# abowman6/CBET_RayTracing_3D

Measured on AMD Instinct MI355X. Metric: ray-steps/sec, OMEGA 60-beam 256^3 sweep, higher is better.
Workload: dtype f64

## Files before the change

cbet_raytracing_3d_amd/build.py:

```python
import os
import shutil
import subprocess
import sys

PKG = os.path.dirname(os.path.abspath(__file__))
ROOT = os.path.dirname(PKG)
CSRC = os.path.join(PKG, "csrc")
LIB_DIR = os.path.join(PKG, "lib")
LIB_PATH = os.path.join(LIB_DIR, "libcbet_mi355x.so")
SOURCES = ["cbet_kernels.hip", "cbet_trace_window.hip", "cbet_trace_exit.hip", "cbet_grid_kernels.hip", "cbet_sph_modes.hip",
           "cbet_target.hip", "cbet_flow.hip", "cbet_abi.cpp", "cbet_host.cpp", "cbet_output.cpp", "cbet_sph_host.cpp", "cbet_target_host.cpp"]
HEADERS = [os.path.join(CSRC, "cbet_device.h"), os.path.join(CSRC, "cbet_relocate.h"), os.path.join(CSRC, "cbet_trace_common.h"), os.path.join(CSRC, "cbet_target_model.h"), os.path.join(ROOT, "include", "cbet_mi355x.h"),
           os.path.join(ROOT, "include", "cbet_omega_beams.h")]

FLAGS = ["-O3", "-std=c++17", "--offload-arch=gfx950", "-ffp-contract=off", "-fPIC", "-shared",
         "-Wall", "-Wextra", "-Wno-unused-result", "-mllvm", "-structurizecfg-skip-uniform-regions=true"]


def hipcc():
    exe = shutil.which("hipcc") or "/opt/rocm/bin/hipcc"
    if not os.path.exists(exe):
        raise RuntimeError("hipcc not found (need ROCm to build the gfx950 library)")
    return exe


def is_stale():
    if not os.path.exists(LIB_PATH):
        return True
    built = os.path.getmtime(LIB_PATH)
    deps = [os.path.join(CSRC, s) for s in SOURCES] + HEADERS + [os.path.abspath(__file__),
                                                                os.path.join(ROOT, "tools", "cbet_gpu.cpp"),
                                                                os.path.join(ROOT, "tools", "cbet_reference_shaped.cpp"),
                                                                os.path.join(ROOT, "include", "cbet_reference_api.hpp")]
    return any(os.path.getmtime(d) > built for d in deps)


def build(force=False, verbose=False, extra_flags=()):
    if not force and not is_stale():
        return LIB_PATH
    os.makedirs(LIB_DIR, exist_ok=True)
    cmd = [hipcc()] + FLAGS + list(extra_flags) + [
        "-I", os.path.join(ROOT, "include"), "-I", CSRC,
        "-o", LIB_PATH] + [os.path.join(CSRC, s) for s in SOURCES] + ["-lrccl"]
    if verbose:
        print(" ".join(cmd), flush=True)
    run = subprocess.run(cmd, stderr=subprocess.PIPE, text=True)
    sys.stderr.write(run.stderr)
    if run.returncode != 0 and "structurizecfg-skip-uniform-regions" in run.stderr:
        print("build: this hipcc does not know -structurizecfg-skip-uniform-regions; building without it", flush=True)
        k = cmd.index("-structurizecfg-skip-uniform-regions=true")
        subprocess.check_call(cmd[:k - 1] + cmd[k + 1:])
    elif run.returncode != 0:
        raise subprocess.CalledProcessError(run.returncode, cmd)
    build_cli(verbose)
    build_ref_shaped(verbose)
    return LIB_PATH


CLI_PATH = os.path.join(PKG, "lib", "cbet-gpu")


def build_cli(verbose=False):
    cmd = ["g++", "-O2", "-std=c++17", "-I", os.path.join(ROOT, "include"),
           os.path.join(ROOT, "tools", "cbet_gpu.cpp"), "-o", CLI_PATH,
           "-L", LIB_DIR, "-lcbet_mi355x", "-Wl,-rpath,$ORIGIN", "-Wl,-rpath-link," + "/opt/rocm/lib"]
    if verbose:
        print(" ".join(cmd), flush=True)
    subprocess.check_call(cmd)
    return CLI_PATH


REF_SHAPED_PATH = os.path.join(PKG, "lib", "cbet-ref-shaped")


def build_ref_shaped(verbose=False):
    cmd = [hipcc(), "-O2", "-std=c++17", "-I", os.path.join(ROOT, "include"),
           os.path.join(ROOT, "tools", "cbet_reference_shaped.cpp"), "-o", REF_SHAPED_PATH,
           "-L", LIB_DIR, "-lcbet_mi355x", "-Wl,-rpath,$ORIGIN"]
    if verbose:
        print(" ".join(cmd), flush=True)
    subprocess.check_call(cmd)
    return REF_SHAPED_PATH


def build_variant(name, extra_flags=(), verbose=False):
    out_dir = os.path.join(ROOT, "build_alt")
    os.makedirs(out_dir, exist_ok=True)
    out = os.path.join(out_dir, "libcbet_%s.so" % name)
    cmd = [hipcc()] + FLAGS + list(extra_flags) + ["-I", os.path.join(ROOT, "include"), "-I", CSRC, "-o", out] + \
        [os.path.join(CSRC, s) for s in SOURCES] + ["-lrccl"]
    if verbose:
        print(" ".join(cmd), flush=True)
    subprocess.check_call(cmd)
    return out


if __name__ == "__main__":
    if len(sys.argv) > 2 and sys.argv[1] == "--variant":
        print(build_variant(sys.argv[2], sys.argv[3:], verbose=True))
    else:
        print(build(force="--force" in sys.argv, verbose=True))
```

cbet_raytracing_3d_amd/csrc/cbet_kernels.hip:

```cpp
#include <hip/hip_runtime.h>

#include "cbet_trace_common.h"

namespace cbet {
namespace {

__device__ __forceinline__ void interp_table2(const double *y1, const double *y2, const double *x, const double xp,
                                              int n, double &o1, double &o2)
{
    const bool ascending = x[0] <= x[n - 1];
    if (ascending ? (xp <= x[0]) : (xp >= x[0])) { o1 = y1[0]; o2 = y2[0]; return; }
    if (ascending ? (xp >= x[n - 1]) : (xp <= x[n - 1])) { o1 = y1[n - 1]; o2 = y2[n - 1]; return; }
    unsigned lo = 0, hi = n - 1, mid = (lo + hi) >> 1;
    while (lo < hi - 1) {
        const bool go_low = ascending ? (x[mid] >= xp) : !(x[mid] <= xp);
        if (go_low) hi = mid; else lo = mid;
        mid = (lo + hi) >> 1;
    }
    const double dx = x[mid + 1] - x[mid], t = xp - x[mid];
    o1 = y1[mid] + (y1[mid + 1] - y1[mid]) / dx * t;
    o2 = y2[mid] + (y2[mid + 1] - y2[mid]) / dx * t;
}

__device__ __forceinline__ void node_plasma(const TabulateArgs &a, const double *s_r, const double *s_ne, const double *s_te,
                                            int i, int j, int k, double &ed, double &kap)
{
    const double xc = i * a.dx + a.xmin, yc = j * a.dy + a.ymin, zc = k * a.dz + a.zmin;
    const double rho = sqrt(xc * xc + yc * yc + zc * zc);
    double etemp;
    interp_table2(s_ne, s_te, s_r, rho, a.nprofile, ed, etemp);
    const double eta = 5.2e-5 * 10.0 / (etemp * sqrt(etemp));
    const double nuei = (1e6 * ed * (kEc * kEc) / kMe) * eta;
    kap = ed / a.ncrit * nuei * a.dt;
}

__global__ void __launch_bounds__(256) k_tabulate(const TabulateArgs a)
{
    extern __shared__ double s_prof[];
    double *s_r = s_prof, *s_ne = s_prof + a.nprofile, *s_te = s_prof + 2 * a.nprofile;
    for (int i = threadIdx.x; i < a.nprofile; i += blockDim.x) {
        s_r[i] = a.r[i];
        s_ne[i] = a.ne[i];
        s_te[i] = a.te[i];
    }
    __syncthreads();
    const long total = (long)a.nx * a.ny * a.nz;
    const long stride = (long)gridDim.x * blockDim.x;
    for (long idx = (long)blockIdx.x * blockDim.x + threadIdx.x; idx < total; idx += stride) {
        const int k = (int)(idx % a.nz);
        const long ij = idx / a.nz;
        const int j = (int)(ij % a.ny);
        const int i = (int)(ij / a.ny);
        double ed, kap;
        node_plasma(a, s_r, s_ne, s_te, i, j, k, ed, kap);
        a.ne3d[idx] = ed;
        a.kap3d[idx] = kap;
    }
}

__global__ void __launch_bounds__(256) k_step_table(const StepTableArgs a)
{
    const long total = (long)a.nx * a.ny * a.nz;
    const long stride = (long)gridDim.x * blockDim.x;
    const long sY = a.nz, sX = (long)a.ny * a.nz;
    for (long idx = (long)blockIdx.x * blockDim.x + threadIdx.x; idx < total; idx += stride) {
        const int k = (int)(idx % a.nz);
        const long ij = idx / a.nz;
        const int j = (int)(ij % a.ny);
        const int i = (int)(ij / a.ny);
        const long oxm = (i == 0) ? 0 : ((i == a.nx - 1) ? -2 * sX : -sX), oxp = (i == 0) ? 2 * sX : ((i == a.nx - 1) ? 0 : sX);
        const long oym = (j == 0) ? 0 : ((j == a.ny - 1) ? -2 * sY : -sY), oyp = (j == 0) ? 2 * sY : ((j == a.ny - 1) ? 0 : sY);
        const long ozm = (k == 0) ? 0 : ((k == a.nz - 1) ? -2 : -1), ozp = (k == 0) ? 2 : ((k == a.nz - 1) ? 0 : 1);
        StepRecord r;
        r.kx = a.xconst * (a.ne3d[idx + oxp] - a.ne3d[idx + oxm]);
        r.ky = a.yconst * (a.ne3d[idx + oyp] - a.ne3d[idx + oym]);
        r.kz = a.zconst * (a.ne3d[idx + ozp] - a.ne3d[idx + ozm]);
        r.kap = a.kap3d[idx];
        a.rec[idx] = r;
    }
}

constexpr int kPrTY = 8, kPrTZ = 64, kPrXC = 16, kPrThreads = 256;
constexpr int kPrPZ = kPrTZ + 2;
constexpr int kPrPlane = (kPrTY + 2) * kPrPZ;
constexpr int kPrTile = kPrTY * kPrTZ;
constexpr int kPrItems = kPrTile + 2 * kPrTZ + 2 * kPrTY;

__global__ void __launch_bounds__(kPrThreads) k_plasma_records(const PlasmaRecordsArgs a)
{
    extern __shared__ double s_prof[];
    const TabulateArgs &t = a.t;
    double *s_r = s_prof, *s_ne = s_prof + t.nprofile, *s_te = s_prof + 2 * t.nprofile;
    double *s_ring = s_prof + 3 * t.nprofile;
    double *s_kap = s_ring + 3 * kPrPlane;
    const int tid = threadIdx.x;
    for (int i = tid; i < t.nprofile; i += kPrThreads) {
        s_r[i] = t.r[i];
        s_ne[i] = t.ne[i];
        s_te[i] = t.te[i];
    }
    __syncthreads();
    const int nx = t.nx, ny = t.ny, nz = t.nz;
    const int k0 = max(0, min((int)blockIdx.x * kPrTZ, nz - kPrTZ));
    const int j0 = max(0, min((int)blockIdx.y * kPrTY, ny - kPrTY));
    const int x0 = (int)blockIdx.z * kPrXC, x1 = min(x0 + kPrXC, nx);
    const int pa = x0 == 0 ? 0 : min(x0 - 1, nx - 3);
    const int pb = x1 == nx ? nx : max(x1 + 1, 3);

    auto emit = [&](int i, int xl, int xh) {
        const double *lo = s_ring + (xl % 3) * kPrPlane, *hi = s_ring + (xh % 3) * kPrPlane, *mid = s_ring + (i % 3) * kPrPlane;
        const double *kap = s_kap + (i % 3) * kPrTile;
        for (int q = tid; q < 2 * kPrTile; q += kPrThreads) {
            const int n = q >> 1, jr = n / kPrTZ, kr = n % kPrTZ;
            const int j = j0 + jr, k = k0 + kr;
            if (j >= ny || k >= nz) continue;
            const int c = (jr + 1) * kPrPZ + kr + 1;
            double v0, v1;
            if ((q & 1) == 0) {
                const int ym = (j == 0) ? 0 : ((j == ny - 1) ? -2 : -1), yp = (j == 0) ? 2 : ((j == ny - 1) ? 0 : 1);
                v0 = a.xconst * (hi[c] - lo[c]);
                v1 = a.yconst * (mid[c + yp * kPrPZ] - mid[c + ym * kPrPZ]);
            } else {
                const int zm = (k == 0) ? 0 : ((k == nz - 1) ? -2 : -1), zp = (k == 0) ? 2 : ((k == nz - 1) ? 0 : 1);
                v0 = a.zconst * (mid[c + zp] - mid[c + zm]);
                v1 = kap[n];
            }
            const long idx = ((long)i * ny + j) * nz + k;
            reinterpret_cast<double2 *>(a.rec + idx)[q & 1] = make_double2(v0, v1);
        }
    };

    for (int p = pa; p < pb; ++p) {
        const bool own_plane = p >= x0 && p < x1;
        double *ring = s_ring + (p % 3) * kPrPlane;
        for (int n = tid; n < (own_plane ? kPrItems : kPrTile); n += kPrThreads) {
            int jj, kk;
            if (n < kPrTile) {
                jj = 1 + n / kPrTZ; kk = 1 + n % kPrTZ;
            } else if (n < kPrTile + 2 * kPrTZ) {
                const int h = n - kPrTile;
                jj = h < kPrTZ ? 0 : kPrTY + 1; kk = 1 + h % kPrTZ;
            } else {
                const int h = n - kPrTile - 2 * kPrTZ;
                kk = h < kPrTY ? 0 : kPrTZ + 1; jj = 1 + h % kPrTY;
            }
            const int j = j0 + jj - 1, k = k0 + kk - 1;
            if (j < 0 || j >= ny || k < 0 || k >= nz) continue;
            double ed, kap;
            if (own_plane && n < kPrTile) {
                node_plasma(t, s_r, s_ne, s_te, p, j, k, ed, kap);
                s_kap[(p % 3) * kPrTile + n] = kap;
                const long idx = ((long)p * ny + j) * nz + k;
                t.ne3d[idx] = ed;
                t.kap3d[idx] = kap;
            } else {
                node_plasma(t, s_r, s_ne, s_te, p, j, k, ed, kap);
            }
            ring[jj * kPrPZ + kk] = ed;
        }
        __syncthreads();
        if (p == 2 && x0 == 0) emit(0, 0, 2);
        if (p - 1 >= 1 && p - 1 >= x0 && p - 1 < x1) emit(p - 1, p - 2, p);
        if (p == nx - 1 && x1 == nx) emit(nx - 1, nx - 3, nx - 1);
        __syncthreads();
    }
}

template <int WL>
struct LdsWindow {
    static constexpr int W = 1 << WL;
    static constexpr int NSLOT = W * W * W;
    double *val;
    unsigned *tag;
    const TraceArgs *args;

    __device__ __forceinline__ unsigned slot(int i, int j, int k) const
    {
        return (unsigned)((((i & (W - 1)) << WL) | (j & (W - 1))) << WL | (k & (W - 1)));
    }
    __device__ __forceinline__ void clear(int lane)
    {
        for (int s = lane; s < NSLOT; s += kWave) {
            val[s] = 0.0;
            tag[s] = kEmptyTag;
        }
    }
    __device__ __forceinline__ void add(unsigned s, double w)
    {
        if (CBET_AUDIT(*args, s < (unsigned)NSLOT))
            __hip_atomic_fetch_add(&val[s], w, __ATOMIC_RELAXED, __HIP_MEMORY_SCOPE_WORKGROUP);
    }
    __device__ __forceinline__ int flush(int lane, double *edep)
    {
        int n = 0;
        for (int s = lane; s < NSLOT; s += kWave) {
            const unsigned t = tag[s];
            if (t != kEmptyTag) {
                global_add(*args, &edep[t], val[s]);
                ++n;
            }
        }
        return n;
    }
};

template <int WL>
__device__ __forceinline__ void lds_deposit8(LdsWindow<WL> &win, bool pending, const unsigned (&slot)[8],
                                             const unsigned (&node)[8], const double (&w)[8],
                                             double *edep, int &n_evict)
{
    unsigned miss = 0;
    if (pending) {
        unsigned t[8];
#pragma unroll
        for (int c = 0; c < 8; ++c)
            t[c] = __hip_atomic_load(&win.tag[slot[c]], __ATOMIC_RELAXED, __HIP_MEMORY_SCOPE_WORKGROUP);
#pragma unroll
        for (int c = 0; c < 8; ++c) {
            if (t[c] == node[c])
                win.add(slot[c], w[c]);
            else
                miss |= 1u << c;
        }
    }
    if (!__any(miss != 0)) return;
    __builtin_amdgcn_wave_barrier();
#pragma unroll
    for (int c = 0; c < 8; ++c) {
        bool pend = (miss >> c) & 1u;
        while (__any(pend)) {
            unsigned t = 0;
            if (pend)
                t = __hip_atomic_load(&win.tag[slot[c]], __ATOMIC_RELAXED, __HIP_MEMORY_SCOPE_WORKGROUP);
            if (pend && t == node[c]) {
                win.add(slot[c], w[c]);
                pend = false;
            }
            __builtin_amdgcn_wave_barrier();
            if (pend) {
                unsigned expect = t;
                const bool won = __hip_atomic_compare_exchange_strong(
                    &win.tag[slot[c]], &expect, node[c], __ATOMIC_RELAXED, __ATOMIC_RELAXED,
                    __HIP_MEMORY_SCOPE_WORKGROUP);
                if (won) {
                    const unsigned long long old = __hip_atomic_exchange(
                        reinterpret_cast<unsigned long long *>(&win.val[slot[c]]),
                        (unsigned long long)__double_as_longlong(w[c]), __ATOMIC_RELAXED,
                        __HIP_MEMORY_SCOPE_WORKGROUP);
                    if (t != kEmptyTag) {
                        global_add(*win.args, &edep[t], __longlong_as_double((long long)old));
                        ++n_evict;
                    }
                    pend = false;
                }
            }
            __builtin_amdgcn_wave_barrier();
        }
    }
}

template <int DEPOSIT>
__global__ void __launch_bounds__(kWave) k_trace_simple(const TraceArgs a)
{
    constexpr int WL = 3;
    constexpr int NSLOT = DEPOSIT == 2 ? (1 << (3 * WL)) : 1;
    __shared__ double s_val[NSLOT];
    __shared__ unsigned s_tag[NSLOT];
    const int lane = threadIdx.x;
    int beam, patch;
    if (!work_item(a, blockIdx.x, beam, patch)) return;
    double *const edep = a.edep + (long)(beam - a.grid_beam0) * a.grid_stride;
    const bool absorb = a.absorption == 1;

    Ray s;
    const int li = patch * kWave + lane;
    const int pre_raynum = li < a.nlive ? a.live[li] : -1;
    bool alive = pre_raynum >= 0;
    if (alive) alive = launch_ray(a, beam, pre_raynum, s);
    const int launched = alive ? 1 : 0;

    const int nx = a.nx, ny = a.ny, nz = a.nz;
    const long sY = nz, sX = (long)ny * nz;
    const int sYh = a.sYh, sXh = a.sXh;
    int nsteps = 0, n_atomics = 0, n_evict = 0;
    unsigned wave_steps = 0;

    LdsWindow<WL> tagged{s_val, s_tag, &a};
    if (DEPOSIT == 2) {
        tagged.clear(lane);
        __syncthreads();
    }

    for (int tt = 0; tt < a.nt; ++tt) {
        if (__ballot(alive) == 0) break;
        ++wave_steps;
        unsigned slot[8] = {0, 0, 0, 0, 0, 0, 0, 0}, node[8] = {0, 0, 0, 0, 0, 0, 0, 0};
        double wgt[8] = {0, 0, 0, 0, 0, 0, 0, 0};
        if (alive) {
            const int im = (s.ci == 0) ? 0 : ((s.ci == nx - 1) ? nx - 3 : s.ci - 1);
            const int ip = (s.ci == 0) ? 2 : ((s.ci == nx - 1) ? nx - 1 : s.ci + 1);
            const int jm = (s.cj == 0) ? 0 : ((s.cj == ny - 1) ? ny - 3 : s.cj - 1);
            const int jp = (s.cj == 0) ? 2 : ((s.cj == ny - 1) ? ny - 1 : s.cj + 1);
            const int km = (s.ck == 0) ? 0 : ((s.ck == nz - 1) ? nz - 3 : s.ck - 1);
            const int kp = (s.ck == 0) ? 2 : ((s.ck == nz - 1) ? nz - 1 : s.ck + 1);
            auto ne_at = [&](int i, int j, int k) { return node_load<true>(a, a.ne3d, (unsigned)(i * sX + j * sY + k)); };
            s.vx -= a.xconst * (ne_at(ip, s.cj, s.ck) - ne_at(im, s.cj, s.ck));
            s.vy -= a.yconst * (ne_at(s.ci, jp, s.ck) - ne_at(s.ci, jm, s.ck));
            s.vz -= a.zconst * (ne_at(s.ci, s.cj, kp) - ne_at(s.ci, s.cj, km));
            s.px += s.vx * a.dt;
            s.py += s.vy * a.dt;
            s.pz += s.vz * a.dt;
            const double fx = (s.px - a.xmin) * a.inv_dx;
            const double fy = (s.py - a.ymin) * a.inv_dy;
            const double fz = (s.pz - a.zmin) * a.inv_dz;
            s.ci = relocate_loop(s.ci, fx, nx);
            s.cj = relocate_loop(s.cj, fy, ny);
            s.ck = relocate_loop(s.ck, fz, nz);
            double inc;
            if (absorb) {
                inc = node_load<true>(a, a.kap3d, (unsigned)(s.ci * sX + s.cj * sY + s.ck)) * s.uray;
                s.uray -= inc;
            } else {
                inc = s.uray;
            }
            const double ox = fx - s.ci - 0.5, oy = fy - s.cj - 0.5, oz = fz - s.ck - 0.5;
            const double dm = 1.0 - fabs(ox), dn = 1.0 - fabs(oy), dl = 1.0 - fabs(oz);
            const int X0 = s.ci + 1, X1 = X0 + (ox < 0 ? -1 : 1);
            const int Y0 = s.cj + 1, Y1 = Y0 + (oy < 0 ? -1 : 1);
            const int Z0 = s.ck + 1, Z1 = Z0 + (oz < 0 ? -1 : 1);
            const double Fx0 = 1.0 - dm, Fy0 = 1.0 - dn, Fz0 = 1.0 - dl;
            const double zy00 = Fz0 * Fy0, zy10 = dl * Fy0, zy01 = Fz0 * dn, zy11 = dl * dn;
            wgt[0] = zy00 * Fx0 * inc; wgt[1] = zy00 * dm * inc; wgt[2] = zy10 * Fx0 * inc; wgt[3] = zy10 * dm * inc;
            wgt[4] = zy01 * Fx0 * inc; wgt[5] = zy01 * dm * inc; wgt[6] = zy11 * Fx0 * inc; wgt[7] = zy11 * dm * inc;
            const int nX0 = X0 * sXh, nX1 = X1 * sXh, nY0 = Y0 * sYh, nY1 = Y1 * sYh;
            node[0] = nX0 + nY0 + Z0; node[1] = nX1 + nY0 + Z0; node[2] = nX0 + nY0 + Z1; node[3] = nX1 + nY0 + Z1;
            node[4] = nX0 + nY1 + Z0; node[5] = nX1 + nY1 + Z0; node[6] = nX0 + nY1 + Z1; node[7] = nX1 + nY1 + Z1;
            if (DEPOSIT == 1) {
#pragma unroll
                for (int c = 0; c < 8; ++c) global_add(a, &edep[node[c]], wgt[c]);
                n_atomics += 8;
            } else {
                slot[0] = tagged.slot(X0, Y0, Z0); slot[1] = tagged.slot(X1, Y0, Z0);
                slot[2] = tagged.slot(X0, Y0, Z1); slot[3] = tagged.slot(X1, Y0, Z1);
                slot[4] = tagged.slot(X0, Y1, Z0); slot[5] = tagged.slot(X1, Y1, Z0);
                slot[6] = tagged.slot(X0, Y1, Z1); slot[7] = tagged.slot(X1, Y1, Z1);
            }
            ++nsteps;
        }
        if (DEPOSIT == 2) lds_deposit8<WL>(tagged, alive, slot, node, wgt, edep, n_evict);
        if (alive) {
            const double *b = a.bounds;
            if (s.uray <= s.ustop || s.px < b[0] || s.px > b[1] || s.py < b[2] || s.py > b[3] || s.pz < b[4] || s.pz > b[5])
                alive = false;
        }
    }
    if (DEPOSIT == 2) {
        __syncthreads();
        n_atomics += tagged.flush(lane, edep) + n_evict;
    }
    const int tot_steps = wave_sum(nsteps), tot_rays = wave_sum(launched), tot_at = wave_sum(n_atomics),
              tot_ev = wave_sum(n_evict);
    if (lane == 0) {
        atomicAdd(&a.counters[kCntSteps], (unsigned long long)tot_steps);
        atomicAdd(&a.counters[kCntRays], (unsigned long long)tot_rays);
        atomicAdd(&a.counters[kCntGlobalAtomics], (unsigned long long)tot_at);
        atomicAdd(&a.counters[kCntEvictions], (unsigned long long)tot_ev);
        atomicAdd(&a.counters[kCntWaveSteps], (unsigned long long)wave_steps);
    }
}

#ifdef CBET_DEBUG_BOUNDS
__device__ unsigned long long g_audit_violations;
#endif

}

hipError_t launch_tabulate(const TabulateArgs &a, hipStream_t stream)
{
    const long total = (long)a.nx * a.ny * a.nz;
    long blocks = (total + 255) / 256;
    if (blocks > 256 * 16) blocks = 256 * 16;
    const size_t lds = sizeof(double) * 3 * (size_t)a.nprofile;
    hipLaunchKernelGGL(k_tabulate, dim3((unsigned)blocks), dim3(256), lds, stream, a);
    return hipGetLastError();
}

hipError_t launch_step_table(const StepTableArgs &a, hipStream_t stream)
{
    const long total = (long)a.nx * a.ny * a.nz;
    long blocks = (total + 255) / 256;
    if (blocks > 256 * 16) blocks = 256 * 16;
    hipLaunchKernelGGL(k_step_table, dim3((unsigned)blocks), dim3(256), 0, stream, a);
    return hipGetLastError();
}

size_t plasma_records_lds(int nprofile)
{
    return sizeof(double) * (3 * (size_t)nprofile + 3 * (size_t)kPrPlane + 3 * (size_t)kPrTile);
}

hipError_t launch_plasma_records(const PlasmaRecordsArgs &a, hipStream_t stream)
{
    const dim3 grid((unsigned)((a.t.nz + kPrTZ - 1) / kPrTZ), (unsigned)((a.t.ny + kPrTY - 1) / kPrTY),
                    (unsigned)((a.t.nx + kPrXC - 1) / kPrXC));
    hipLaunchKernelGGL(k_plasma_records, grid, dim3(kPrThreads), plasma_records_lds(a.t.nprofile), stream, a);
    return hipGetLastError();
}

hipError_t audit_violations(unsigned long long *out, bool reset, hipStream_t stream)
{
#ifdef CBET_DEBUG_BOUNDS
    hipError_t e = hipStreamSynchronize(stream);
    if (e != hipSuccess) return e;
    e = hipMemcpyFromSymbol(out, HIP_SYMBOL(g_audit_violations), sizeof *out);
    if (e == hipSuccess && reset) {
        const unsigned long long zero = 0;
        e = hipMemcpyToSymbol(HIP_SYMBOL(g_audit_violations), &zero, sizeof zero);
    }
    return e;
#else
    (void)out; (void)reset; (void)stream;
    return hipErrorNotSupported;
#endif
}

hipError_t launch_trace(const TraceArgs &a0, int variant, bool force_idx64, hipStream_t stream)
{
    TraceArgs a = a0;
#ifdef CBET_DEBUG_BOUNDS
    {
        const long cells = (long)(a.nx + 2) * a.sXh;
        a.audit_lo = a.edep;
        a.audit_hi = a.edep + (a.grid_stride ? a.grid_stride * (long)(a.beam_lo - a.grid_beam0 + a.nbeams_local) : cells);
        if (a.quantity != 0) a.audit_hi = a.edep + 4 * a.comp_stride;
        a.audit_nodes = (unsigned long long)a.nx * a.ny * a.nz;
        a.audit_hsize = (unsigned long long)a.hsize;
        hipError_t e = hipGetSymbolAddress((void **)&a.audit_count, HIP_SYMBOL(g_audit_violations));
        if (e != hipSuccess) return e;
    }
#endif
    if (variant == CBET_KERNEL_LDS_WINDOW) return launch_trace_window(a, force_idx64, stream);
    if (variant == kTraceExits) return launch_trace_exit(a, force_idx64, stream);
    const long waves = a.item_count;
    if (waves <= 0) return hipSuccess;
    const dim3 grid((unsigned)waves);
    if (variant == CBET_KERNEL_GLOBAL_ATOMICS) hipLaunchKernelGGL((k_trace_simple<1>), grid, dim3(kWave), 0, stream, a);
    else hipLaunchKernelGGL((k_trace_simple<2>), grid, dim3(kWave), 0, stream, a);
    return hipGetLastError();
}

}
```

Before: 167.3 billion.

## Replace binary-search profile interpolation with binned lookup and precomputed slopes

In the plasma-records kernel, the per-node binary search over the radial profile is replaced by a 1024-bin start-index table plus a short linear walk, with segment slopes precomputed in LDS. Halo nodes now compute only density, and the x/y squared terms are hoisted per plane. A fallback to the old search is kept for non-monotonic or degenerate profiles. It uses more LDS and adds setup work per block. Precomputed slopes change rounding slightly compared with the divide-per-lookup form.

```diff
diff --git a/cbet_raytracing_3d_amd/build.py b/cbet_raytracing_3d_amd/build.py
--- a/cbet_raytracing_3d_amd/build.py
+++ b/cbet_raytracing_3d_amd/build.py
@@ -10,7 +10,7 @@
 LIB_PATH = os.path.join(LIB_DIR, "libcbet_mi355x.so")
 SOURCES = ["cbet_kernels.hip", "cbet_trace_window.hip", "cbet_trace_exit.hip", "cbet_grid_kernels.hip", "cbet_sph_modes.hip",
            "cbet_target.hip", "cbet_flow.hip", "cbet_abi.cpp", "cbet_host.cpp", "cbet_output.cpp", "cbet_sph_host.cpp", "cbet_target_host.cpp"]
-HEADERS = [os.path.join(CSRC, "cbet_device.h"), os.path.join(CSRC, "cbet_relocate.h"), os.path.join(CSRC, "cbet_trace_common.h"), os.path.join(CSRC, "cbet_target_model.h"), os.path.join(ROOT, "include", "cbet_mi355x.h"),
+HEADERS = [os.path.join(CSRC, "cbet_device.h"), os.path.join(CSRC, "cbet_relocate.h"), os.path.join(CSRC, "cbet_profile_search.h"), os.path.join(CSRC, "cbet_trace_common.h"), os.path.join(CSRC, "cbet_target_model.h"), os.path.join(ROOT, "include", "cbet_mi355x.h"),
            os.path.join(ROOT, "include", "cbet_omega_beams.h")]
 
 FLAGS = ["-O3", "-std=c++17", "--offload-arch=gfx950", "-ffp-contract=off", "-fPIC", "-shared",
diff --git a/cbet_raytracing_3d_amd/csrc/cbet_kernels.hip b/cbet_raytracing_3d_amd/csrc/cbet_kernels.hip
--- a/cbet_raytracing_3d_amd/csrc/cbet_kernels.hip
+++ b/cbet_raytracing_3d_amd/csrc/cbet_kernels.hip
@@ -1,5 +1,6 @@
 #include <hip/hip_runtime.h>
 
+#include "cbet_profile_search.h"
 #include "cbet_trace_common.h"
 
 namespace cbet {
@@ -85,21 +86,63 @@
 constexpr int kPrPlane = (kPrTY + 2) * kPrPZ;
 constexpr int kPrTile = kPrTY * kPrTZ;
 constexpr int kPrItems = kPrTile + 2 * kPrTZ + 2 * kPrTY;
+constexpr int kPrDoubles = 3 * kPrPlane + 3 * kPrTile;
+
+__device__ __forceinline__ void records_node_plasma(const TabulateArgs &a, const ProfileTables &prof, bool direct, double xy,
+                                                    int k, double &ed, double &kap)
+{
+    const double zc = k * a.dz + a.zmin;
+    const double rho = sqrt(xy + zc * zc);
+    double etemp;
+    if (direct) profile_interp2(prof, rho, ed, etemp);
+    else interp_table2(prof.y1, prof.y2, prof.x, rho, a.nprofile, ed, etemp);
+    const double eta = 5.2e-5 * 10.0 / (etemp * sqrt(etemp));
+    const double nuei = (1e6 * ed * (kEc * kEc) / kMe) * eta;
+    kap = ed / a.ncrit * nuei * a.dt;
+}
+
+__device__ __forceinline__ double records_node_ne(const TabulateArgs &a, const ProfileTables &prof, bool direct, double xy, int k)
+{
+    const double zc = k * a.dz + a.zmin;
+    const double rho = sqrt(xy + zc * zc);
+    if (direct) return profile_interp1(prof, rho);
+    double ed, etemp;
+    interp_table2(prof.y1, prof.y2, prof.x, rho, a.nprofile, ed, etemp);
+    return ed;
+}
 
 __global__ void __launch_bounds__(kPrThreads) k_plasma_records(const PlasmaRecordsArgs a)
 {
     extern __shared__ double s_prof[];
     const TabulateArgs &t = a.t;
-    double *s_r = s_prof, *s_ne = s_prof + t.nprofile, *s_te = s_prof + 2 * t.nprofile;
-    double *s_ring = s_prof + 3 * t.nprofile;
+    const int np = t.nprofile;
+    double *s_r = s_prof, *s_ne = s_prof + np, *s_te = s_prof + 2 * np;
+    double *s_sne = s_prof + 3 * np, *s_ste = s_prof + 4 * np;
+    double *s_ring = s_prof + 5 * np;
     double *s_kap = s_ring + 3 * kPrPlane;
+    unsigned short *s_start = reinterpret_cast<unsigned short *>(s_kap + 3 * kPrTile);
+    int *s_direct = reinterpret_cast<int *>(s_start + kProfileBins);
     const int tid = threadIdx.x;
-    for (int i = tid; i < t.nprofile; i += kPrThreads) {
+    for (int i = tid; i < np; i += kPrThreads) {
         s_r[i] = t.r[i];
         s_ne[i] = t.ne[i];
         s_te[i] = t.te[i];
     }
+    if (tid == 0) *s_direct = 1;
     __syncthreads();
+    ProfileTables prof;
+    prof.x = s_r; prof.y1 = s_ne; prof.y2 = s_te; prof.s1 = s_sne; prof.s2 = s_ste; prof.start = s_start;
+    prof.x0 = s_r[0]; prof.xn = s_r[np - 1]; prof.scale = profile_bin_scale(s_r, np); prof.n = np;
+    if (tid == 0 && !profile_scale_ok(prof.scale)) *s_direct = 0;
+    for (int m = tid; m < np - 1; m += kPrThreads) {
+        if (!profile_pair_ok(s_r, m)) *s_direct = 0;
+        const double dx = s_r[m + 1] - s_r[m];
+        s_sne[m] = (s_ne[m + 1] - s_ne[m]) / dx;
+        s_ste[m] = (s_te[m + 1] - s_te[m]) / dx;
+        profile_fill_bins(s_r, np, prof.x0, prof.scale, m, s_start);
+    }
+    __syncthreads();
+    const bool direct = *s_direct != 0;
     const int nx = t.nx, ny = t.ny, nz = t.nz;
     const int k0 = max(0, min((int)blockIdx.x * kPrTZ, nz - kPrTZ));
     const int j0 = max(0, min((int)blockIdx.y * kPrTY, ny - kPrTY));
@@ -133,6 +176,7 @@
     for (int p = pa; p < pb; ++p) {
         const bool own_plane = p >= x0 && p < x1;
         double *ring = s_ring + (p % 3) * kPrPlane;
+        const double xc = p * t.dx + t.xmin, xx = xc * xc;
         for (int n = tid; n < (own_plane ? kPrItems : kPrTile); n += kPrThreads) {
             int jj, kk;
             if (n < kPrTile) {
@@ -146,15 +190,17 @@
             }
             const int j = j0 + jj - 1, k = k0 + kk - 1;
             if (j < 0 || j >= ny || k < 0 || k >= nz) continue;
-            double ed, kap;
+            const double yc = j * t.dy + t.ymin, xy = xx + yc * yc;
+            double ed;
             if (own_plane && n < kPrTile) {
-                node_plasma(t, s_r, s_ne, s_te, p, j, k, ed, kap);
+                double kap;
+                records_node_plasma(t, prof, direct, xy, k, ed, kap);
                 s_kap[(p % 3) * kPrTile + n] = kap;
                 const long idx = ((long)p * ny + j) * nz + k;
                 t.ne3d[idx] = ed;
                 t.kap3d[idx] = kap;
             } else {
-                node_plasma(t, s_r, s_ne, s_te, p, j, k, ed, kap);
+                ed = records_node_ne(t, prof, direct, xy, k);
             }
             ring[jj * kPrPZ + kk] = ed;
         }
@@ -396,7 +442,7 @@
 
 size_t plasma_records_lds(int nprofile)
 {
-    return sizeof(double) * (3 * (size_t)nprofile + 3 * (size_t)kPrPlane + 3 * (size_t)kPrTile);
+    return sizeof(double) * (5 * (size_t)nprofile + (size_t)kPrDoubles) + sizeof(unsigned short) * kProfileBins + sizeof(double);
 }
 
 hipError_t launch_plasma_records(const PlasmaRecordsArgs &a, hipStream_t stream)
diff --git a/cbet_raytracing_3d_amd/csrc/cbet_profile_search.h b/cbet_raytracing_3d_amd/csrc/cbet_profile_search.h
--- /dev/null
+++ b/cbet_raytracing_3d_amd/csrc/cbet_profile_search.h
@@ -0,0 +1,76 @@
+#ifndef CBET_PROFILE_SEARCH_H_
+#define CBET_PROFILE_SEARCH_H_
+
+#include <math.h>
+
+#if defined(__HIPCC__)
+#define CBET_PS_HD __host__ __device__ __forceinline__
+#else
+#define CBET_PS_HD static inline
+#endif
+
+namespace cbet {
+
+constexpr int kProfileBins = 1024;
+
+CBET_PS_HD double profile_bin_scale(const double *x, int n) { return (double)kProfileBins / (x[n - 1] - x[0]); }
+
+CBET_PS_HD bool profile_scale_ok(double scale) { return scale > 0.0 && scale < HUGE_VAL; }
+
+CBET_PS_HD bool profile_pair_ok(const double *x, int i) { return x[i] < x[i + 1]; }
+
+CBET_PS_HD int profile_bin(double xp, double x0, double scale)
+{
+    return (int)fmin(fmax((xp - x0) * scale, 0.0), (double)(kProfileBins - 1));
+}
+
+CBET_PS_HD void profile_fill_bins(const double *x, int n, double x0, double scale, int m, unsigned short *start)
+{
+    const int lo = m == 0 ? 0 : profile_bin(x[m], x0, scale) + 1;
+    const int hi = m == n - 2 ? kProfileBins - 1 : profile_bin(x[m + 1], x0, scale);
+    for (int b = lo; b <= hi; ++b) start[b] = (unsigned short)m;
+}
+
+CBET_PS_HD int profile_segment(const double *x, const unsigned short *start, double x0, double scale, double xp, double &xm)
+{
+    int m = start[profile_bin(xp, x0, scale)];
+    double lo = x[m], hi = x[m + 1];
+    while (hi < xp) {
+        lo = hi;
+        ++m;
+        hi = x[m + 1];
+    }
+    xm = lo;
+    return m;
+}
+
+struct ProfileTables {
+    const double *x, *y1, *y2;
+    const double *s1, *s2;
+    const unsigned short *start;
+    double x0, xn, scale;
+    int n;
+};
+
+CBET_PS_HD double profile_interp1(const ProfileTables &t, double xp)
+{
+    if (xp <= t.x0) return t.y1[0];
+    if (xp >= t.xn) return t.y1[t.n - 1];
+    double xm;
+    const int m = profile_segment(t.x, t.start, t.x0, t.scale, xp, xm);
+    return t.y1[m] + t.s1[m] * (xp - xm);
+}
+
+CBET_PS_HD void profile_interp2(const ProfileTables &t, double xp, double &o1, double &o2)
+{
+    if (xp <= t.x0) { o1 = t.y1[0]; o2 = t.y2[0]; return; }
+    if (xp >= t.xn) { o1 = t.y1[t.n - 1]; o2 = t.y2[t.n - 1]; return; }
+    double xm;
+    const int m = profile_segment(t.x, t.start, t.x0, t.scale, xp, xm);
+    const double u = xp - xm;
+    o1 = t.y1[m] + t.s1[m] * u;
+    o2 = t.y2[m] + t.s2[m] * u;
+}
+
+}
+#endif
```

Measured after the change: 168.1 billion, median of 6. Within noise of the previous version (+0.5%).
